# jenkinsm13/julia-spira

Measured on AMD Instinct MI355X. Metric: Msamples/sec at 1920x1080 spp=64 depth=8; fraction of HBM roofline, higher is better.
Workload: dtype f64

## Files before the change

julia-spira_amd/csrc/spira_device.h:

```cpp
#pragma once
#include <hip/hip_runtime.h>
#include <stdint.h>
#include <type_traits>
#include "spira_fastdiv.h"

namespace spira {

__device__ __forceinline__ float sqrt_rn(float x) { return __builtin_sqrtf(x); }
__device__ __forceinline__ double sqrt_rn(double x) { return __builtin_sqrt(x); }

constexpr int kBlock = 256;
#ifndef SPIRA_WAVES_F32
#define SPIRA_WAVES_F32 5
#endif
#ifndef SPIRA_WAVES_F64
#define SPIRA_WAVES_F64 4
#endif
#define SPIRA_WAVES_PER_SIMD(T) (sizeof(T) == 8 ? SPIRA_WAVES_F64 : SPIRA_WAVES_F32)
constexpr uint32_t kMaxTries = 64;

template <class T> struct Vec { T x, y, z; };

template <class T> __device__ __forceinline__ Vec<T> mk(T x, T y, T z) { Vec<T> r; r.x = x; r.y = y; r.z = z; return r; }
template <class T> __device__ __forceinline__ Vec<T> operator+(Vec<T> a, Vec<T> b) { return mk<T>(a.x + b.x, a.y + b.y, a.z + b.z); }
// ... 1117 lines not shown
            if (have) {
                const uint32_t *kw = reinterpret_cast<const uint32_t *>(&s_rnd[e]);
                k.hA = kw[0]; k.hB = kw[1]; k.hBr = (k.hB << 16) | (k.hB >> 16);
            }
            while (__any(have)) {
                bool done = false;
                if (have) {
                    T u0, u1, u2;
                    rng3<T>(k, t, u0, u1, u2, (T)(1.0 / 1048576.0));
                    Vec<T> c = mk<T>(u0, u1, u2) - mk<T>(1, 1, 1);
                    done = dot(c, c) < (T)1.0;
                    if (!done && t == kMaxTries) { c = mk<T>(0, 0, 0); done = true; }
                    if (done) { Pack4<T> w; w.x = c.x; w.y = c.y; w.z = c.z; w.w = 0; s_rnd[e] = w; }
                    ++t;
                }
                const unsigned long long m = __ballot(done);
                if (done) {
                    e = next + __popcll(m & lt_mask); t = 1;
                    have = e < n_list;
                    if (have) {
                        const uint32_t *kw = reinterpret_cast<const uint32_t *>(&s_rnd[e]);
                        k.hA = kw[0]; k.hB = kw[1]; k.hBr = (k.hB << 16) | (k.hB >> 16);
                    }
                }
                next += (uint32_t)__popcll(m);
            }
        }
        wave_lds_sync();
#pragma unroll
        for (int r = 0; r < R; ++r) {
            const bool alive = pend[r].kind != kDead;
            const unsigned long long m = __ballot(alive);
            if (alive) {
                Vec<T> rnd = mk<T>(0, 0, 0);
                if (pend[r].kind != kMirror) { const Pack4<T> w = s_rnd[ent[r]]; rnd = mk<T>(w.x, w.y, w.z); }
                const Vec<T> nd = segment_back<T>(o[r], pend[r], rnd);
                const uint32_t dst = region + fill + __popcll(m & lt_mask);
                Pack4<T> A, B; Pack2<T> C;
                A.x = o[r].x; A.y = o[r].y; A.z = o[r].z; A.w = nd.x;
                B.x = nd.y; B.y = nd.z; B.z = beta[r].x; B.w = beta[r].y;
                C.x = beta[r].z; C.y = Bits<T>::from_u32(q[r]);
                a.qout.A[dst] = A; a.qout.B[dst] = B; a.qout.C[dst] = C;
            }
            fill += (uint32_t)__popcll(m);
        }
        wave_lds_sync();
    }
    for (int sft = 32; sft > 0; sft >>= 1) { n_rmw += __shfl_down(n_rmw, sft); n_seg += __shfl_down(n_seg, sft); n_store += __shfl_down(n_store, sft); }
    if (lane == 0) {
        if (scatter) a.cnt_out[wid] = fill;
        a.blk_stats[4 * wid] = n_seg;
        a.blk_stats[4 * wid + 1] = n_rmw;
        a.blk_stats[4 * wid + 2] = n_store;
        a.blk_stats[4 * wid + 3] = FIRST ? 0u : n_seg;
    }
}

template <class T> struct PathArgs {
    SceneGlobal<T> scene;
    RenderConst<T> rc;
    RayQueue<T> q[2];
    uint32_t *qref[2];
    uint2 *qkey[2];
    uint32_t cam_consts;
    Pack3<T> *L;
    uint32_t *blk_stats;
    uint32_t cap;
    uint32_t pass;
    uint32_t n_first;
    uint32_t dense_pct;
    Pack4<T> *mesh_list;
    uint32_t mesh_min_batch;
    uint32_t refill_free;
    uint32_t mesh_mode;
    uint32_t *mesh_count;
    uint32_t resume_k, resume_nw;
    uint32_t *redo;
    uint32_t redo_only;
    Stats *stats;
    Pack4<T> *accum;
    FastDiv fd_keff;
    uint32_t k_eff;
    uint32_t accum_first;
};

#ifndef SPIRA_RESOLVE_RUN
#define SPIRA_RESOLVE_RUN 4
#endif
__device__ __forceinline__ uint32_t owned_pixel(uint32_t w, uint32_t nw, uint32_t l) {
    constexpr uint32_t kRun = SPIRA_RESOLVE_RUN;
    static_assert(64 % kRun == 0, "a run length divides the wave");
    return ((l / kRun) * nw + w) * kRun + l % kRun;
}

template <class T>
__device__ __forceinline__ void resolve_pixel(Pack4<T> *accum, const Pack3<T> *L, uint32_t tile_pixels, uint32_t k_eff, bool first_pass, uint32_t p) {
    Pack4<T> acc;
    if (first_pass) { acc.x = 0; acc.y = 0; acc.z = 0; acc.w = 0; } else acc = accum[p];
    uint32_t s = 0;
    for (; s + 8 <= k_eff; s += 8) {
        Pack3<T> l[8];
#pragma unroll
        for (int k = 0; k < 8; ++k) l[k] = L[(size_t)(s + k) * tile_pixels + p];
#pragma unroll
        for (int k = 0; k < 8; ++k) { acc.x = acc.x + l[k].x; acc.y = acc.y + l[k].y; acc.z = acc.z + l[k].z; }
    }
    for (; s < k_eff; ++s) {
        const Pack3<T> l = L[(size_t)s * tile_pixels + p];
        acc.x = acc.x + l.x; acc.y = acc.y + l.y; acc.z = acc.z + l.z;
    }
    accum[p] = acc;
}

__device__ __forceinline__ float pack_qref(uint32_t q, uint32_t, float) { return __uint_as_float(q); }
__device__ __forceinline__ double pack_qref(uint32_t q, uint32_t ref, double) { return __longlong_as_double((long long)((unsigned long long)q | ((unsigned long long)ref << 32))); }
__device__ __forceinline__ uint32_t unpack_q(float w) { return __float_as_uint(w); }
__device__ __forceinline__ uint32_t unpack_q(double w) { return (uint32_t)(unsigned long long)__double_as_longlong(w); }
__device__ __forceinline__ uint32_t unpack_ref(double w) { return (uint32_t)((unsigned long long)__double_as_longlong(w) >> 32); }

#ifdef SPIRA_MESH_STATS
__device__ unsigned long long g_mesh_dbg[32];
#define MESH_STAT(...) __VA_ARGS__
#else
#define MESH_STAT(...)
#endif

#ifndef SPIRA_CARRY_KEY
#define SPIRA_CARRY_KEY 1
#endif
#ifndef SPIRA_WAVES_B_F32
#define SPIRA_WAVES_B_F32 4
#endif
#ifndef SPIRA_WAVES_B_F64
#define SPIRA_WAVES_B_F64 SPIRA_WAVES_F64
#endif
#ifndef SPIRA_WAVES_PATH_F32
#define SPIRA_WAVES_PATH_F32 6
#endif
template <class T, int R, bool BVH, bool EXT, bool SPEC, int MODE = 0, bool TRI = true>
__global__ __launch_bounds__(kBlock, MODE == 2 ? (sizeof(T) == 8 ? SPIRA_WAVES_B_F64 : SPIRA_WAVES_B_F32) : (sizeof(T) == 4 ? SPIRA_WAVES_PATH_F32 : SPIRA_WAVES_F64)) void k_path(const PathArgs<T> a) {
    extern __shared__ __attribute__((aligned(32))) unsigned char lds_raw[];
    constexpr uint32_t WPB = kBlock / 64, SUB = 64 * R;
    constexpr bool kRefArray = sizeof(T) == 4;
    constexpr bool kCarry = SPIRA_CARRY_KEY && !BVH && !EXT;
    constexpr uint32_t kStageShift = 25, kRefMask = (1u << kStageShift) - 1u;
    const uint32_t lane = threadIdx.x & 63, wave = threadIdx.x >> 6;
    const uint32_t NW = gridDim.x * WPB, wid = blockIdx.x * WPB + wave;
    const RenderConst<T> &rc = a.rc;
    using Pol = typename std::conditional<SPEC, SpecDiv, ExactDiv>::type;
    Pol pol;
    if (!SPEC && a.redo_only) {
        uint32_t any = 0;
        for (uint32_t w = 0; w < WPB; ++w) any |= a.redo[blockIdx.x * WPB + w];
        if (!any) return;
    }
    T *cam_lds = reinterpret_cast<T *>(lds_raw + scene_lds_bytes<T>(a.scene.n_spheres, a.scene.n_materials, a.scene.n_triangles) + WPB * SUB * sizeof(Pack4<T>));
    if (threadIdx.x < 12) {
        const Vec<T> *cv = threadIdx.x < 3 ? &rc.cam_origin : (threadIdx.x < 6 ? &rc.cam_llc : (threadIdx.x < 9 ? &rc.cam_hor : &rc.cam_ver));
        const uint32_t cc = threadIdx.x % 3;
        cam_lds[threadIdx.x] = cc == 0 ? cv->x : (cc == 1 ? cv->y : cv->z);
    }
    Pack4<T> *cam_sph = reinterpret_cast<Pack4<T> *>(reinterpret_cast<unsigned char *>(cam_lds) + 128);
    constexpr bool kCam = !EXT;
    if (kCam && MODE != 2 && a.cam_consts)
        for (uint32_t i = threadIdx.x; i < a.scene.n_spheres; i += blockDim.x) {
            const T *sp = a.scene.spheres5 + 5 * (size_t)i;
            const Vec<T> oc = rc.cam_origin - mk<T>(sp[0], sp[1], sp[2]);
            Pack4<T> k; k.x = oc.x; k.y = oc.y; k.z = oc.z; k.w = dot(oc, oc) - sp[3] * sp[3];
            cam_sph[i] = k;
        }
    const SceneLds<T> sc = stage_scene<T>(a.scene, lds_raw);
    const PixelDiv<T> pix_div = pixel_divisors<T>(rc);
    if (!SPEC && a.redo_only) {
        if (!a.redo[wid]) return;
        if (lane == 0) atomicAdd(&a.stats->redone_waves, 1ull);
    }
    Pack4<T> *s_rnd = reinterpret_cast<Pack4<T> *>(lds_raw + scene_lds_bytes<T>(a.scene.n_spheres, a.scene.n_materials, a.scene.n_triangles)) + wave * SUB;
    constexpr uint32_t mesh_mode = BVH ? (uint32_t)MODE : 0u;
    const uint32_t kseg = mesh_mode == 2u ? a.resume_k : 1u;
    if (mesh_mode == 2u && wid * kseg >= a.resume_nw) return;
    const uint32_t region = wid * kseg * a.cap;
    const unsigned long long lt_mask = (1ull << lane) - 1ull;
    const uint32_t ref_base = sc.n_spheres + sc.n_triangles;
    const bool mixed = mesh_mode != 0u || rc.max_depth <= 128u;
    const uint32_t dense_pct = mixed ? a.dense_pct : 0u;
    const bool defer = mesh_mode != 0u || (BVH && mixed && a.mesh_list != nullptr);
    Pack4<T> *mlist = a.mesh_list + 3 * (size_t)region;
    uint32_t n_rmw = 0, n_store = 0, n_seg = 0, n_enq = 0, n_park = 0;
    uint32_t n_wtrips = 0, n_ltrips = 0;
    uint32_t n_in = 0;
    const bool own = !BVH && !EXT && !TRI && sizeof(T) == 8 && a.accum != nullptr;
    const uint32_t n_own = own ? 64u * a.k_eff : 0u;
    const uint32_t n_sub_first = own ? (n_own + SUB - 1) / SUB : (a.n_first + SUB - 1) / SUB;

    auto park = [&](uint32_t slot_i, const Vec<T> o_, const Vec<T> d_, const Vec<T> beta_, T closest_, uint32_t q_, int prim_, uint32_t stage_hit) {
        Pack4<T> A, B, C;
        A.x = o_.x; A.y = o_.y; A.z = o_.z; A.w = d_.x;
        B.x = d_.y; B.y = d_.z; B.z = beta_.x; B.w = beta_.y;
        C.x = beta_.z; C.y = closest_; C.z = Bits<T>::from_u32(q_); C.w = Bits<T>::from_u32((uint32_t)(prim_ + 1) | (stage_hit << kStageShift));
        mlist[3 * (size_t)slot_i] = A; mlist[3 * (size_t)slot_i + 1] = B; mlist[3 * (size_t)slot_i + 2] = C;
    };
    uint32_t mfill = 0;
    constexpr int kMaxSeg = 16;
    uint32_t pfx[kMaxSeg + 1];
    bool segmented = false;
    {
        uint32_t cnt = 0;
        if (mesh_mode == 2u && lane < kseg && wid * kseg + lane < a.resume_nw) cnt = a.mesh_count[wid * kseg + lane];
        pfx[0] = 0;
#pragma unroll
        for (int j = 0; j < kMaxSeg; ++j) pfx[j + 1] = pfx[j] + (uint32_t)__builtin_amdgcn_readlane((int)cnt, j);
        if (mesh_mode == 2u) { mfill = pfx[kMaxSeg]; segmented = true; }
    }
    const uint32_t first_sub = own ? 0u : (mesh_mode == 1u ? (wid % a.resume_k) * (NW / a.resume_k) + wid / a.resume_k : wid);
    const uint32_t sub_step = own ? 1u : NW;
    MESH_STAT(unsigned long long dbg_t0 = __builtin_readcyclecounter(); unsigned long long dbg_sess = 0, dbg_walk = 0; uint32_t dbg_ns = 0, dbg_ws = 0, dbg_ls = 0, dbg_rf = 0, dbg_rays = 0, dbg_rounds = 0, dbg_ws1 = 0, dbg_ls1 = 0, dbg_h[4] = {0, 0, 0, 0};)
    for (uint32_t round = 0; ; ++round) {
        MESH_STAT(++dbg_rounds;)
        const bool first = mesh_mode != 2u && round == 0;
        const RayQueue<T> qin = a.q[(round + 1) & 1], qout = a.q[round & 1];
        const uint32_t *rin = a.qref[(round + 1) & 1];
        uint32_t *rout = a.qref[round & 1];
        const uint2 *kin = a.qkey[(round + 1) & 1];
        uint2 *kout = a.qkey[round & 1];
        const uint32_t limit = first ? (own ? n_own : a.n_first) : n_in;
        const uint32_t n_sub = first ? n_sub_first : (n_in + SUB - 1) / SUB;
        uint32_t fill = 0;
        for (uint32_t sub = first ? first_sub : 0u; sub < n_sub; sub += first ? sub_step : 1u) {
            Vec<T> o[R], beta[R];
            Pending<T> pend[R];
            ExtState<T> ex[R];
            uint32_t q[R], ent[R], stg[R], ref[R];
            uint32_t ka[R], kb[R];
            bool valid[R];
#pragma unroll
            for (int r = 0; r < R; ++r) {
                const uint32_t idx = sub * SUB + r * 64 + lane;
                valid[r] = false; stg[r] = round; ref[r] = 0; q[r] = 0; ka[r] = 0; kb[r] = 0;
                pend[r].kind = kDead; pend[r].rough = 0; pend[r].v = mk<T>(0, 0, 0);
                o[r] = mk<T>(0, 0, 0); beta[r] = mk<T>(1, 1, 1);
                bool parked = false; T park_t = 0; int park_prim = -1;
                uint32_t qf = idx;
                bool in = idx < limit;
                if (own && first) {
                    const uint32_t t = idx / SPIRA_RESOLVE_RUN, run = fastdiv(t, a.fd_keff);
                    const uint32_t px = owned_pixel(wid, NW, run * SPIRA_RESOLVE_RUN + idx % SPIRA_RESOLVE_RUN);
                    qf = (t - run * a.k_eff) * rc.tile_pixels + px;
                    in = in && px < rc.tile_pixels;
                }
                if (in) {
                    if (first) {
                        uint32_t pixel, sample, pi, pj;
                        Vec<T> d;
                        q[r] = qf;
                        path_of<T>(rc, qf, a.pass, pi, pj, pixel, sample);
                        if (kCarry) { ka[r] = mix32(rc.sA + pixel) ^ (sample << 8); kb[r] = mix32(rc.sB ^ pixel) + (sample << 8); }
                        camera_ray_lds<T>(rc, cam_lds, pix_div, pi, pj, pixel, sample, o[r], d, pol);
                        if (EXT) { ex[r].flags = rc.flags; if (rc.flags & kExtSpectral) beta[r] = ext_wavelength<T>(sc, rc.sA, rc.sB, pixel, sample, ex[r]); }
                        T t; uint32_t slot = 0;
                        int prim;
                        if (defer) {
                            if (kCam && a.cam_consts) closest_hit_local<T, Pol, TRI, true>(sc, o[r], d, (T)0.001, t, prim, pol, cam_sph);
                            else closest_hit_local<T, Pol, TRI>(sc, o[r], d, (T)0.001, t, prim, pol);
                            parked = mesh_box_hit<T>(sc, o[r], d, t);
                        } else if (kCam && !BVH && a.cam_consts) { closest_hit_local<T, Pol, TRI, true>(sc, o[r], d, (T)0.001, t, prim, pol, cam_sph); }
                        else prim = closest_hit<T, BVH, Pol, TRI>(sc, o[r], d, (T)0.001, t, slot, pol);
                        ++n_seg;
                        if (parked) { park_t = t; park_prim = prim; pend[r].v = d; }
                        else if (prim < 0) {
                            const Vec<T> c = sky_term_x<T, EXT>(d, beta[r], &ex[r]);
                            Pack3<T> l; l.x = c.x; l.y = c.y; l.z = c.z;
                            a.L[qf] = l;
                            ++n_store;
                        } else {
                            valid[r] = true;
                            o[r] = o[r] + d * t;
                            ref[r] = (BVH && prim >= (int)ref_base) ? ref_base + slot : (uint32_t)prim;
                            pend[r].v = d;
                        }
                    } else {
                        const Pack4<T> A = qin.A[region + idx], B = qin.B[region + idx];
                        const Pack2<T> C = qin.C[region + idx];
                        o[r] = mk<T>(A.x, A.y, A.z);
                        pend[r].v = mk<T>(A.w, B.x, B.y);
                        beta[r] = mk<T>(B.z, B.w, C.x);
                        q[r] = unpack_q(C.y);
                        uint32_t w;
                        if constexpr (kRefArray) w = rin[region + idx]; else w = unpack_ref(C.y);
                        if (mixed) { stg[r] = w >> kStageShift; ref[r] = w & kRefMask; } else ref[r] = w;
                        if (kCarry) { const uint2 k = kin[region + idx]; ka[r] = k.x; kb[r] = k.y; }
                        valid[r] = true;
                    }
                }
                if (defer && first) {
                    const unsigned long long mp = __ballot(parked);
                    if (parked) park(mfill + __popcll(mp & lt_mask), o[r], pend[r].v, beta[r], park_t, q[r], park_prim, 0u);
                    mfill += (uint32_t)__popcll(mp); n_park += (uint32_t)__popcll(mp);
                }
            }
            while (true) {
                uint32_t n_list = 0, n_valid = 0;
#pragma unroll
                for (int r = 0; r < R; ++r) {
                    bool want = false;
                    RngKey key;
                    const Vec<T> d = pend[r].v;
                    pend[r].kind = kDead;
                    if (valid[r]) {
                        uint32_t pixel = 0, sample = 0, pi, pj;
                        const bool scatter = stg[r] + 1 < rc.max_depth;
                        int prim = (int)ref[r]; uint32_t slot = 0;
                        if (BVH && ref[r] >= ref_base) { prim = (int)ref_base; slot = ref[r] - ref_base; }
                        const uint32_t qi = q[r] & 0x7FFFFFFFu;
                        const bool has_l = (q[r] >> 31) != 0;
                        if (EXT) {
                            path_of<T>(rc, qi, a.pass, pi, pj, pixel, sample);
                            ex[r].flags = rc.flags;
                            if (rc.flags & kExtSpectral) (void)ext_wavelength<T>(sc, rc.sA, rc.sB, pixel, sample, ex[r]);
                        }
                        Vec<T> contrib;
                        const bool has_contrib = shade_hit<T, BVH, EXT, Pol, TRI>(sc, o[r], d, prim, slot, beta[r], scatter, contrib, pend[r], &ex[r], pol);
                        if (has_contrib) {
                            Pack3<T> l; l.x = contrib.x; l.y = contrib.y; l.z = contrib.z;
                            if (has_l) { const Pack3<T> l0 = a.L[qi]; l.x = l0.x + contrib.x; l.y = l0.y + contrib.y; l.z = l0.z + contrib.z; ++n_rmw; }
                            else ++n_store;
                            a.L[qi] = l;
                            q[r] |= 0x80000000u;
                        } else if (!scatter && !has_l) {
                            Pack3<T> l; l.x = 0; l.y = 0; l.z = 0;
                            a.L[qi] = l;
                            ++n_store;
                        }
                        want = (pend[r].kind == kDiffuse || pend[r].kind == kSpecRough);
                        if (want || (EXT && pend[r].kind == kDielectric)) {
                            if (kCarry && mixed) {
                                key.hA = mix32(ka[r] ^ stg[r]); key.hB = mix32(kb[r] + stg[r]); key.hBr = (key.hB << 16) | (key.hB >> 16);
                            } else {
                                if (!EXT) path_of<T>(rc, qi, a.pass, pi, pj, pixel, sample);
                                key = rng_key(rc.sA, rc.sB, pixel, sample, stg[r]);
                            }
                            if (EXT && pend[r].kind == kDielectric) dielectric_resolve<T>(pend[r], d, key);
                        }
                    }
                    const unsigned long long mv = __ballot(pend[r].kind != kDead);
                    n_valid += (uint32_t)__popcll(mv);
                    const unsigned long long m = __ballot(want);
                    if (want) {
                        ent[r] = n_list + __popcll(m & lt_mask);
                        uint32_t *kw = reinterpret_cast<uint32_t *>(&s_rnd[ent[r]]);
                        kw[0] = key.hA; kw[1] = key.hB;
                    }
                    n_list += (uint32_t)__popcll(m);
                }
                if (n_valid == 0) break;
                wave_lds_sync();
// ... 237 lines not shown
                    if (prim < 0) {
                        const uint32_t qi = q_ & 0x7FFFFFFFu;
                        ExtState<T> ex1; ex1.flags = rc.flags; ex1.bR = 0; ex1.bG = 0; ex1.bB = 0;
                        if (EXT && (rc.flags & kExtSpectral)) {
                            uint32_t pi, pj, pixel, sample;
                            path_of<T>(rc, qi, a.pass, pi, pj, pixel, sample);
                            (void)ext_wavelength<T>(sc, rc.sA, rc.sB, pixel, sample, ex1);
                        }
                        const Vec<T> c = sky_term_x<T, EXT>(d_, beta_, &ex1);
                        Pack3<T> l; l.x = c.x; l.y = c.y; l.z = c.z;
                        if (q_ >> 31) { const Pack3<T> l0 = a.L[qi]; l.x = l0.x + c.x; l.y = l0.y + c.y; l.z = l0.z + c.z; ++n_rmw; }
                        else ++n_store;
                        a.L[qi] = l;
                    } else {
                        const Vec<T> hp = o_ + d_ * closest;
                        const uint32_t w_ = ((prim >= (int)ref_base) ? ref_base + slot : (uint32_t)prim) | (stage_hit << kStageShift);
                        const uint32_t dst = region + fill + __popcll(mh & lt_mask);
                        Pack4<T> A, B; Pack2<T> C;
                        A.x = hp.x; A.y = hp.y; A.z = hp.z; A.w = d_.x;
                        B.x = d_.y; B.y = d_.z; B.z = beta_.x; B.w = beta_.y;
                        C.x = beta_.z; C.y = pack_qref(q_, w_, (T)0);
                        qout.A[dst] = A; qout.B[dst] = B; qout.C[dst] = C;
                        if constexpr (kRefArray) rout[dst] = w_;
                    }
                }
                fill += (uint32_t)__popcll(mh);
                finished = false;
                const unsigned long long mf = __ballot(!walking);
                const uint32_t take = min((uint32_t)__popcll(mf), mfill - next);
                if (!walking && (uint32_t)__popcll(mf & lt_mask) < take) {
                    const uint32_t e = next + (uint32_t)__popcll(mf & lt_mask);
                    const Pack4<T> *ent = mlist + 3 * (size_t)e;
                    if (segmented) {
                        uint32_t seg = 0, off = e;
#pragma unroll
                        for (int j = 1; j < kMaxSeg; ++j) if (e >= pfx[j]) { seg = (uint32_t)j; off = e - pfx[j]; }
                        ent = a.mesh_list + 3 * ((size_t)(wid * kseg + seg) * a.cap + off);
                    }
                    const Pack4<T> A = ent[0], B = ent[1], C = ent[2];
                    o_ = mk<T>(A.x, A.y, A.z); d_ = mk<T>(A.w, B.x, B.y); beta_ = mk<T>(B.z, B.w, C.x);
                    closest = C.y;
                    q_ = Bits<T>::to_u32(C.z);
                    const uint32_t pw = Bits<T>::to_u32(C.w);
                    prim = (int)(pw & kRefMask) - 1;
                    stage_hit = pw >> kStageShift;
                    slot = 0;
                    T t0;
                    if (bvh8_enter<T>(sc, o_, d_, closest, ry, t0)) { bvh8_begin<T>(wk, ry, t0, (T)0.001, sc.bvh_root[2].w); walking = true; }
                    else finished = true;
                }
                next += take;
                if (!__any(walking)) { if (__any(finished)) continue; break; }
                const bool more = next < mfill;
                MESH_STAT(++dbg_rf; const unsigned long long dbg_w0 = __builtin_readcyclecounter();)
                uint32_t n_now = (uint32_t)__popcll(__ballot(walking));
                while (true) {
                    ++n_wtrips; n_ltrips += n_now;
                    MESH_STAT(++dbg_ws; { const uint32_t nl = (uint32_t)__popcll(__ballot(walking)); dbg_ls += nl; if (segmented) { ++dbg_ws1; dbg_ls1 += nl; } ++dbg_h[nl <= 8 ? 0 : (nl <= 24 ? 1 : (nl <= 48 ? 2 : 3))]; })
                    if (walking && !bvh8_step<T, kLdsStack>(sc, wk, ry, o_, d_, (T)0.001, (int)ref_base, closest, prim, slot, lstack, stack, lane)) { walking = false; finished = true; }
                    const uint32_t n_walk = (uint32_t)__popcll(__ballot(walking));
                    n_now = n_walk;
                    if (n_walk == 0 || (more && 64u - n_walk >= a.refill_free)) break;
                }

                MESH_STAT(dbg_walk += __builtin_readcyclecounter() - dbg_w0;)
            }
            }
            mfill = 0;
            segmented = false;
            MESH_STAT(dbg_sess += __builtin_readcyclecounter() - dbg_s0;)
        }
        n_in = fill;
        n_enq += fill;
        if (n_in == 0 && (mfill == 0 || mesh_mode == 1u)) break;
        __builtin_amdgcn_fence(__ATOMIC_RELEASE, "workgroup");
        __builtin_amdgcn_fence(__ATOMIC_ACQUIRE, "workgroup");
    }
    for (int sft = 32; sft > 0; sft >>= 1) { n_rmw += __shfl_down(n_rmw, sft); n_seg += __shfl_down(n_seg, sft); n_store += __shfl_down(n_store, sft); }
    const bool again = SPEC && __any(outside_window<T>(pol));
    if (own && !again && !(SPEC && a.redo_only == 2u)) {
        __builtin_amdgcn_fence(__ATOMIC_RELEASE, "workgroup");
        __builtin_amdgcn_fence(__ATOMIC_ACQUIRE, "workgroup");
        const uint32_t px = owned_pixel(wid, NW, lane);
        if (px < rc.tile_pixels) resolve_pixel<T>(a.accum, a.L, rc.tile_pixels, a.k_eff, a.accum_first != 0, px);
        const uint32_t seg = __shfl(n_seg, 0), rmw = __shfl(n_rmw, 0), sto = __shfl(n_store, 0);
        if (lane < 4) {
            unsigned long long *f = lane == 0 ? &a.stats->segments : (lane == 1 ? &a.stats->rays_enqueued : (lane == 2 ? &a.stats->radiance_rmw : &a.stats->radiance_store));
            atomicAdd(f, (unsigned long long)(lane == 0 ? seg : (lane == 1 ? n_enq : (lane == 2 ? rmw : sto))));
        }
    }
    MESH_STAT(if (lane == 0) { unsigned long long *g = g_mesh_dbg + (mesh_mode == 2u ? 16 : 0);
                               atomicAdd(&g[0], __builtin_readcyclecounter() - dbg_t0); atomicAdd(&g[1], dbg_sess); atomicAdd(&g[2], (unsigned long long)dbg_ns);
                               atomicAdd(&g[3], (unsigned long long)dbg_ws); atomicAdd(&g[4], (unsigned long long)dbg_ls); atomicAdd(&g[5], (unsigned long long)dbg_rf);
                               atomicAdd(&g[6], (unsigned long long)dbg_rays); atomicAdd(&g[7], (unsigned long long)dbg_rounds); atomicAdd(&g[9], dbg_walk); atomicAdd(&g[10], 1ull); atomicAdd(&g[11], (unsigned long long)dbg_ws1); atomicAdd(&g[12], (unsigned long long)dbg_ls1);
                               atomicAdd(&g[8], (unsigned long long)dbg_h[0]); atomicAdd(&g[13], (unsigned long long)dbg_h[1]); atomicAdd(&g[14], (unsigned long long)dbg_h[2]); atomicAdd(&g[15], (unsigned long long)dbg_h[3]); })
    if (lane == 0) {
        if (mesh_mode == 2u) {
            const uint32_t row = 4 * wid * kseg;
            a.blk_stats[row] += n_seg; a.blk_stats[row + 1] += n_rmw; a.blk_stats[row + 2] += n_store; a.blk_stats[row + 3] += n_enq;
        } else {
            a.blk_stats[4 * wid] = n_seg;
            a.blk_stats[4 * wid + 1] = n_rmw;
            a.blk_stats[4 * wid + 2] = n_store;
            a.blk_stats[4 * wid + 3] = n_enq;
            if (mesh_mode == 1u) a.mesh_count[wid] = mfill;
        }
        if (SPEC) a.redo[wid] = again ? 1u : 0u;
        if (BVH && n_park && !again && !(SPEC && a.redo_only == 2u)) atomicAdd(&a.stats->rays_parked, (unsigned long long)n_park);
        if (BVH && mesh_mode != 1u && n_wtrips && !again && !(SPEC && a.redo_only == 2u)) { atomicAdd(&a.stats->mesh_wave_trips, (unsigned long long)n_wtrips); atomicAdd(&a.stats->mesh_lane_trips, (unsigned long long)n_ltrips); }
    }
}

template <class T, bool BVH, bool EXT>
__global__ __launch_bounds__(kBlock) void k_mega(const BounceArgs<T> a) {
    extern __shared__ __attribute__((aligned(32))) unsigned char lds_raw[];
    const SceneLds<T> sc = stage_scene<T>(a.scene, lds_raw);
    const RenderConst<T> &rc = a.rc;
    unsigned long long nseg = 0;
    const uint32_t stride = gridDim.x * kBlock;
    uint32_t idx = blockIdx.x * kBlock + threadIdx.x;
    bool fresh = true;
    uint32_t pixel = 0, sample = 0, b = 0;
    Vec<T> o = mk<T>(0, 0, 0), d = mk<T>(0, 0, 1), beta = mk<T>(1, 1, 1), Lacc = mk<T>(0, 0, 0);
    ExtState<T> ex; ex.flags = rc.flags; ex.bR = 0; ex.bG = 0; ex.bB = 0;
    while (idx < a.n_first) {
        if (fresh) {
            uint32_t pi, pj;
            path_of<T>(rc, idx, a.pass, pi, pj, pixel, sample);
            camera_ray<T>(rc, pi, pj, pixel, sample, o, d);
            beta = mk<T>(1, 1, 1); Lacc = mk<T>(0, 0, 0); b = 0;
            if (EXT && (rc.flags & kExtSpectral)) beta = ext_wavelength<T>(sc, rc.sA, rc.sB, pixel, sample, ex);
            fresh = false;
        }
        Vec<T> contrib; T t_hit;
        SegInfo si = trace_segment<T, BVH, EXT>(sc, rc, o, d, beta, pixel, sample, b, b + 1 < rc.max_depth, contrib, t_hit, &ex);
        ++nseg;
        if (b == 0) { if (si.has_contrib) Lacc = contrib; }
        else if (si.has_contrib) Lacc = Lacc + contrib;
        ++b;
        if (!si.alive || b == rc.max_depth) {
            Pack3<T> l; l.x = Lacc.x; l.y = Lacc.y; l.z = Lacc.z;
            a.L[idx] = l;
            idx += stride;
            fresh = true;
        }
    }
    for (int sft = 32; sft > 0; sft >>= 1) nseg += __shfl_down(nseg, sft);
    if ((threadIdx.x & 63) == 0 && nseg) atomicAdd(&a.stats->segments, nseg);
}

template <class T, bool BVH, bool EXT>
__global__ __launch_bounds__(64) void k_trace(const BounceArgs<T> a, const uint32_t *ijs, uint32_t n_paths, int *prims, T *ts,
                                              T *dirs, T *radiance) {
    extern __shared__ __attribute__((aligned(32))) unsigned char lds_raw[];
    const SceneLds<T> sc = stage_scene<T>(a.scene, lds_raw);
    const RenderConst<T> &rc = a.rc;
    uint32_t p = blockIdx.x * blockDim.x + threadIdx.x;
    if (p >= n_paths) return;
    uint32_t i = ijs[3 * p], j = ijs[3 * p + 1], sample = ijs[3 * p + 2];
    uint32_t pixel = (j - 1) * rc.width + (i - 1);
    Vec<T> o, d, beta = mk<T>(1, 1, 1), Lacc = mk<T>(0, 0, 0);
    camera_ray<T>(rc, i, j, pixel, sample, o, d);
    ExtState<T> ex; ex.flags = rc.flags; ex.bR = 0; ex.bG = 0; ex.bB = 0;
    if (EXT && (rc.flags & kExtSpectral)) beta = ext_wavelength<T>(sc, rc.sA, rc.sB, pixel, sample, ex);
    for (uint32_t b = 0; b < rc.max_depth; ++b) {
        Vec<T> contrib; T t_hit;
        Vec<T> dir_in = d;
// ... 761 lines not shown
```

julia-spira_amd/csrc/spira_hip.hip:

```cpp
#include <hip/hip_runtime.h>
#include <sys/mman.h>
#include <rccl/rccl.h>
#include <dlfcn.h>

#include <algorithm>
#include <atomic>
#include <chrono>
#include <cmath>
#include <cstdio>
#include <cstdlib>
#include <cstring>
#include <condition_variable>
#include <mutex>
#include <new>
#include <string>
#include <thread>
#include <vector>

#include "../../include/spira_hip.h"
#include "../../include/spira_spd.h"
#include "spira_device.h"
#include "spira_bvh.h"
#include "spira_validate.h"

// ... 493 lines not shown
                  const spira_params *p, spira::SceneGlobal<T> &g, bool reuse = false) {
    if (h) { scene_pointers<T>(h->store, g); return 0; }
    if (reuse) { scene_pointers<T>(c.scene, g); return 0; }
    const uint32_t nt = triangles10 ? p->n_triangles : 0;
    if (int rc = scene_upload<T>(c.scene, st, c.have_done ? c.ev_done : nullptr, spheres5, materials8, triangles10, p->n_spheres, p->n_materials, nt)) return rc;
    scene_pointers<T>(c.scene, g);
    return 0;
}

template <class T>
int attach_spd(Ctx &c, hipStream_t st, const spira_params *p, spira::SceneGlobal<T> &g) {
    g.spd = nullptr;
    if (!(p->flags & SPIRA_EXT_SPECTRAL)) return 0;
    DevBuf &b = sizeof(T) == 4 ? c.spd32 : c.spd64;
    if (!b.p) {
        static_assert(SPIRA_SPD_N == spira::kSpdN && SPIRA_SPD_ROWS == spira::kSpdRows, "SPD table shape");
        T host[SPIRA_SPD_ROWS * SPIRA_SPD_N];
        for (int r = 0; r < SPIRA_SPD_ROWS; ++r)
            for (int i = 0; i < SPIRA_SPD_N; ++i) host[r * SPIRA_SPD_N + i] = (T)spira_spd_table[r][i];
        if (int rc = b.ensure(sizeof host)) return rc;
        HIP_TRY(hipMemcpy(b.p, host, sizeof host, hipMemcpyHostToDevice));
    }
    (void)st;
    g.spd = (const T *)b.p;
    return 0;
}

template <class T>
int check_handle(const spira_scene *h) {
    if (!h || h->magic != kSceneMagic) return fail(SPIRA_E_INVALID, "scene handle is NULL or was destroyed");
    if (h->prec != (int)sizeof(T)) return fail(SPIRA_E_INVALID, "scene handle was created in the other precision");
    if (h->device != tl_device) return fail(SPIRA_E_INVALID, "scene handle belongs to another device (spira_set_device)");
    return 0;
}

struct PathPlan {
    uint64_t waves = 0;
    uint64_t packets = 0;
    uint64_t batch = 0;
    bool queues = false;
    bool mesh = false;
    bool two_pass = false;
    bool spec = false;
};
template <class T>
int ensure_path_plan(Ctx &c, const PathPlan &pl) {
    using P4 = spira::Pack4<T>;
    using P2 = spira::Pack2<T>;
    if (pl.queues)
        for (int i = 0; i < 2; ++i) {
            if (int rc = c.qA[i].ensure(pl.packets * sizeof(P4))) return rc;
            if (int rc = c.qB[i].ensure(pl.packets * sizeof(P4))) return rc;
            if (int rc = c.qC[i].ensure(pl.packets * sizeof(P2))) return rc;
            if (sizeof(T) == 4) { if (int rc = c.qR[i].ensure(pl.packets * sizeof(uint32_t))) return rc; }
            if (!pl.mesh) { if (int rc = c.qK[i].ensure(pl.packets * sizeof(uint2))) return rc; }
        }
    if (pl.mesh) { if (int rc = c.mesh_list.ensure(3 * pl.packets * sizeof(P4))) return rc; }
    if (pl.two_pass) { if (int rc = c.mesh_count.ensure(pl.waves * sizeof(uint32_t))) return rc; }
    if (pl.spec) { if (int rc = c.redo.ensure(pl.waves * sizeof(uint32_t))) return rc; }
    if (int rc = c.blkstats.ensure(pl.waves * 4 * sizeof(uint32_t))) return rc;
    if (int rc = c.L.ensure(pl.batch * sizeof(spira::Pack3<T>))) return rc;
    return c.stats.ensure(sizeof(spira::Stats));
}
template <class T>
int verify_path_args(const Ctx &c, const spira::PathArgs<T> &a, uint32_t first_launch_blocks) {
    using P4 = spira::Pack4<T>;
    using P2 = spira::Pack2<T>;
    const uint64_t nw = (uint64_t)first_launch_blocks * (spira::kBlock / 64), n = nw * a.cap;
    auto covers = [](const DevBuf &b, const void *ptr, uint64_t bytes) { return ptr == b.p && b.p != nullptr && b.cap >= bytes; };
    const char *bad = nullptr;
    const bool mesh = a.scene.n_bvh_tris != 0;
    if ((uint64_t)a.n_first > n) bad = "the pass does not fit its queue regions";
    if (a.rc.max_depth > 1 || mesh)
        for (int i = 0; i < 2 && !bad; ++i) {
            if (!covers(c.qA[i], a.q[i].A, n * sizeof(P4)) || !covers(c.qB[i], a.q[i].B, n * sizeof(P4)) || !covers(c.qC[i], a.q[i].C, n * sizeof(P2))) bad = "hit queues";
            else if (sizeof(T) == 4 && !covers(c.qR[i], a.qref[i], n * sizeof(uint32_t))) bad = "hit reference arrays";
            else if (!mesh && !covers(c.qK[i], a.qkey[i], n * sizeof(uint2))) bad = "carried RNG keys";
        }
    if (!bad && a.mesh_list && !covers(c.mesh_list, a.mesh_list, 3 * n * sizeof(P4))) bad = "mesh lists";
    if (!bad && a.mesh_mode != 0 && (!a.mesh_list || !covers(c.mesh_count, a.mesh_count, nw * sizeof(uint32_t)) || a.resume_k == 0 || a.resume_k > 16 || nw % a.resume_k != 0 || a.resume_nw != nw))
        bad = "parked-ray counts of a two-launch mesh pass";
    if (!bad && a.redo && !covers(c.redo, a.redo, nw * sizeof(uint32_t))) bad = "redo flags";
    if (!bad && !covers(c.blkstats, a.blk_stats, nw * 4 * sizeof(uint32_t))) bad = "per-wave statistics";
    if (!bad && !covers(c.L, a.L, (uint64_t)a.n_first * sizeof(spira::Pack3<T>))) bad = "per-path radiance";
    if (!bad && !covers(c.stats, a.stats, sizeof(spira::Stats))) bad = "counters";
    if (!bad && a.accum) {
        const uint64_t tp = a.rc.tile_pixels;
        if (!covers(c.accum, a.accum, tp * sizeof(spira::Pack4<T>)) || sizeof(T) != 8 || a.scene.n_triangles || mesh || (a.rc.flags & (SPIRA_EXT_DIELECTRIC | SPIRA_EXT_SPECTRAL)) ||
            a.k_eff == 0 || a.k_eff > 64 || (uint64_t)a.k_eff * tp != a.n_first || 64 * nw < tp || a.cap < 64ull * a.k_eff)
            bad = "pixel-owning pass";
    }
    if (bad) return fail(SPIRA_E_LIMIT, std::string("internal: a workspace is smaller than the launch needs (") + bad + ")");
    return 0;
}

template <class T>
int render_impl(const spira_scene *h, const T *spheres5, const T *materials8, const T *triangles10, const T *camera12, const spira_params *p,
                T *out_hdr, T *out_img, bool out_on_device, void *user_stream,
                bool progressive = false, uint32_t sample0 = 0, uint32_t *rng_states = nullptr, const SlabCtl *slab = nullptr) {
    uint32_t rows = 0;
    const bool cont = slab && slab->index > 0;
    if (!p) return fail(SPIRA_E_INVALID, "params is NULL");
    tl_lds_optin = hipSuccess;
    Lap lap("render");
    if (h) { if (int rc = check_handle<T>(h)) return rc; }
    else if (!cont) { if (int rc = validate_scene<T>(spheres5, materials8, triangles10, p->n_spheres, p->n_materials, triangles10 ? p->n_triangles : 0)) return rc; }
    if (int rc = validate_params(camera12, p, h ? h->store.nt : (triangles10 ? p->n_triangles : 0), &rows)) return rc;
    lap("validate");
    if (!out_hdr && !out_img) return fail(SPIRA_E_INVALID, "both outputs are NULL");
    if (progressive && (uint64_t)sample0 + p->spp > SPIRA_MAX_SPP) return fail(SPIRA_E_LIMIT, "sample0 + spp exceeds 2^24");
    if (progressive && (p->flags & SPIRA_SEM_MASK) == SPIRA_SEM_HYBRID) return fail(SPIRA_E_UNSUPPORTED, "SPIRA_SEM_HYBRID has no accumulate entry (its image is a mean of tone-mapped samples)");
    if (progressive && (p->flags & SPIRA_SEM_MASK) == SPIRA_SEM_METAL && sample0 > 0 && !rng_states)
        return fail(SPIRA_E_INVALID, "SPIRA_SEM_METAL with sample0 > 0 needs rng_states (the LCG states the previous call left); "
                                     "without them every call would replay the samples of the first");
    Ctx *cp = nullptr;
    if (int rc = get_ctx(&cp)) return rc;
    Ctx &c = *cp;
    std::lock_guard<std::recursive_mutex> lock(c.mu);
    hipStream_t st = out_on_device ? (hipStream_t)user_stream : c.stream;
    if (int rc = order_after_previous(c, st)) return rc;
    lap("context");

    const uint32_t W = p->width;
    const uint64_t tile_pixels = (uint64_t)rows * W;
    uint32_t target = p->batch_rays ? p->batch_rays : env_u32("SPIRA_BATCH_RAYS", 160u << 20);
    uint64_t slots64 = std::max<uint64_t>(1, target / tile_pixels);
    slots64 = std::min<uint64_t>(slots64, p->spp);
    slots64 = (p->spp + (p->spp + slots64 - 1) / slots64 - 1) / ((p->spp + slots64 - 1) / slots64);
    if (slots64 * tile_pixels > 0x7FFFFFFFull) return fail(SPIRA_E_LIMIT, "tile too large: rows*width must be < 2^31");
    const uint32_t slots = (uint32_t)slots64;
    const uint64_t batch = slots64 * tile_pixels;
    const uint32_t sem = p->flags & SPIRA_SEM_MASK;
    const bool mega = (p->flags & SPIRA_KERNEL_MASK) == SPIRA_KERNEL_MEGA || sem != SPIRA_SEM_A;
    const bool metal_wavefront = sem == SPIRA_SEM_METAL && (p->flags & SPIRA_KERNEL_MASK) == SPIRA_KERNEL_WAVEFRONT;
    uint64_t metal_launches = 0;
    const bool per_bounce = !mega && (p->flags & SPIRA_KERNEL_MASK) == SPIRA_KERNEL_BOUNCE;
    const bool persistent = !mega && !per_bounce;
    const bool profile = ((p->flags & SPIRA_FLAG_PROFILE) != 0 && per_bounce) || persistent;
    int R = (int)env_u32("SPIRA_R", 2);
    if (R != 1 && R != 2) R = 2;
    if (p->flags & (SPIRA_EXT_DIELECTRIC | SPIRA_EXT_SPECTRAL)) R = 2;

    const uint32_t nt_scene = h ? h->store.nt : (triangles10 ? p->n_triangles : 0);
    const bool mesh_two_pass = persistent && nt_scene > SPIRA_LDS_TRIANGLES && p->max_depth <= 128 && env_u32("SPIRA_DEFER_MESH", 1) && env_u32("SPIRA_MESH_TWO_PASS", 1);
    const uint32_t blocks_per_cu = !persistent ? 16 : ((nt_scene > SPIRA_LDS_TRIANGLES && !mesh_two_pass) ? 4 : 32);
    const uint32_t max_blocks = (uint32_t)c.num_cus * env_u32("SPIRA_BLOCKS_PER_CU", blocks_per_cu);
    const uint32_t wpb = spira::kBlock / 64;
    const uint32_t sub = 64 * R;
    const bool fused = persistent && sizeof(T) == 8 && R == 2 && nt_scene == 0 && (p->flags & (SPIRA_EXT_DIELECTRIC | SPIRA_EXT_SPECTRAL)) == 0 &&
                       slots <= 64 && env_u32("SPIRA_FUSED_RESOLVE", 1) != 0;
    auto geometry = [&](uint64_t n_first, uint32_t &G, uint32_t &cap) {
        if (fused) {
            const uint64_t k = n_first / tile_pixels;
            G = (uint32_t)((tile_pixels + 64 * wpb - 1) / (64 * wpb));
            cap = (uint32_t)((64 * k + sub - 1) / sub * sub);
            return;
        }
        const uint64_t n_sub = (n_first + sub - 1) / sub;
        G = (uint32_t)std::min<uint64_t>((n_sub + wpb - 1) / wpb, max_blocks);
        const uint64_t nw = (uint64_t)G * wpb;
        cap = (uint32_t)(((n_sub + nw - 1) / nw) * sub);
    };
    uint32_t G_max = 0, cap_max = 0;
    geometry(batch, G_max, cap_max);
    const uint64_t q_rays = (uint64_t)cap_max * G_max * wpb;
    if (q_rays > 0xFFFFFFFFull) return fail(SPIRA_E_LIMIT, "pass too large");

    using P4 = spira::Pack4<T>;
    using P2 = spira::Pack2<T>;
    const bool mesh_scene = nt_scene > SPIRA_LDS_TRIANGLES;
    const bool defer_mesh = persistent && mesh_scene && p->max_depth <= 128 && env_u32("SPIRA_DEFER_MESH", 1) != 0;
    PathPlan plan;
    plan.waves = (uint64_t)G_max * wpb; plan.packets = q_rays; plan.batch = batch;
    plan.queues = !mega && (p->max_depth > 1 || (persistent && mesh_scene));
    plan.mesh = defer_mesh; plan.two_pass = defer_mesh && mesh_two_pass; plan.spec = persistent && env_u32("SPIRA_SPEC_DIV", 1) != 0;
    if (persistent) { if (int rc = ensure_path_plan<T>(c, plan)) return rc; }
    else {
        if (plan.queues)
            for (int i = 0; i < 2; ++i) {
                if (int rc = c.qA[i].ensure(q_rays * sizeof(P4))) return rc;
                if (int rc = c.qB[i].ensure(q_rays * sizeof(P4))) return rc;
                if (int rc = c.qC[i].ensure(q_rays * sizeof(P2))) return rc;
            }
        if (sem != SPIRA_SEM_HYBRID) { if (int rc = c.L.ensure(batch * sizeof(spira::Pack3<T>))) return rc; }
        if (per_bounce) { if (int rc = c.counts.ensure((size_t)(p->max_depth + 2) * G_max * wpb * sizeof(uint32_t))) return rc; }
        if (int rc = c.blkstats.ensure((size_t)(per_bounce ? p->max_depth + 1 : 1) * G_max * wpb * 4 * sizeof(uint32_t))) return rc;
        if (int rc = c.stats.ensure(sizeof(spira::Stats))) return rc;
    }
    if (int rc = c.accum.ensure(tile_pixels * sizeof(P4))) return rc;

    lap("workspaces");
    spira::BounceArgs<T> a{};
    if (int rc = acquire_scene<T>(c, st, h, spheres5, materials8, triangles10, p, a.scene, cont)) return rc;
    if (int rc = attach_spd<T>(c, st, p, a.scene)) return rc;
    lap("scene");
    const bool scene_moderate = h ? h->store.moderate : c.scene.moderate;
    fill_const<T>(a.rc, camera12, p, rows, slots);
    if (!fastdiv_selfcheck(a.rc.tile_pixels, (uint32_t)batch) || !fastdiv_selfcheck(a.rc.width, a.rc.tile_pixels) ||
        !fastdiv_selfcheck(a.rc.stripe_h ? a.rc.stripe_h : 1, rows))
        return fail(SPIRA_E_LIMIT, "internal: fast division self-check failed");
    a.L = (spira::Pack3<T> *)c.L.p;
    a.stats = (spira::Stats *)c.stats.p;

    const size_t lds = spira::scene_lds_bytes<T>(a.scene.n_spheres, a.scene.n_materials, a.scene.n_triangles);
    const uint32_t n_pass = (p->spp + slots - 1) / slots;

    T *d_hdr = out_hdr, *d_img = out_img;
    if (!out_on_device) {
        size_t plane3 = 3 * tile_pixels * sizeof(T);
        if (int rc = c.out_tmp.ensure(2 * plane3)) return rc;
        d_hdr = out_hdr ? (T *)c.out_tmp.p : nullptr;
        d_img = out_img ? (T *)((char *)c.out_tmp.p + plane3) : nullptr;
    }

    size_t n_prof = 0;
    if (profile) {
        n_prof = (size_t)n_pass * (persistent ? 1 : std::max<uint32_t>(p->max_depth, 1)) * 2;
        if (int rc = profile_events(c, (cont ? c.ev_used : 0) + n_prof)) return rc;
    }
    if (!cont) {
        c.ev_used = 0;
        c.ev_mid_used = 0;
        HIP_TRY(hipMemsetAsync(c.stats.p, 0, sizeof(spira::Stats), st));
        HIP_TRY(hipEventRecord(c.ev_start, st));
    }
    uint64_t launches = 0;

    a.rc.sample0 = progressive ? sample0 : 0;
    uint32_t *d_rng = nullptr;
    if (progressive) {
        const uint32_t lblocks = std::min<uint32_t>((uint32_t)((tile_pixels + spira::kBlock - 1) / spira::kBlock), max_blocks);
        if (!out_on_device) HIP_TRY(hipMemcpyAsync(d_hdr, out_hdr, 3 * tile_pixels * sizeof(T), hipMemcpyHostToDevice, st));
        hipLaunchKernelGGL((spira::k_load_accum<T>), dim3(lblocks), dim3(spira::kBlock), 0, st, (P4 *)c.accum.p, (const T *)d_hdr, (uint32_t)tile_pixels);
        ++launches;
        if (rng_states) {
            d_rng = rng_states;
            if (!out_on_device) {
                if (int rc = c.rng.ensure(tile_pixels * sizeof(uint32_t))) return rc;
                d_rng = (uint32_t *)c.rng.p;
                if (sample0 > 0) HIP_TRY(hipMemcpyAsync(d_rng, rng_states, tile_pixels * sizeof(uint32_t), hipMemcpyHostToDevice, st));
            }
        }
    }

    if (p->max_depth == 0) {
        if (!progressive) HIP_TRY(hipMemsetAsync(c.accum.p, 0, tile_pixels * sizeof(P4), st));
    } else if (sem == SPIRA_SEM_HYBRID) {
        const uint64_t P = tile_pixels;
        if (P > 0xFFFFFFFFull / 2) return fail(SPIRA_E_LIMIT, "image too large for SPIRA_SEM_HYBRID");
        if (int rc = c.hyb_state.ensure(12 * P * sizeof(T))) return rc;
        if (int rc = c.hyb_mat.ensure(P * sizeof(uint32_t))) return rc;
        if (int rc = c.rng.ensure(P * sizeof(uint32_t))) return rc;
        const size_t n_flags = (size_t)p->spp * (p->max_depth + 1);
        if (int rc = c.hyb_flags.ensure(n_flags * sizeof(uint32_t))) return rc;
        HIP_TRY(hipMemsetAsync(c.hyb_flags.p, 0, n_flags * sizeof(uint32_t), st));
        HIP_TRY(hipMemsetAsync(c.accum.p, 0, P * sizeof(P4), st));
// ... 56 lines not shown
        hipLaunchKernelGGL(spira::k_fold_stats, dim3(1), dim3(64), 0, st, (const uint32_t *)c.blkstats.p, Gm * wpb, (spira::Stats *)c.stats.p);
        launches += 2;
        metal_launches = 1;
    } else if (sem == SPIRA_SEM_METAL) {
        uint32_t blocks = std::min<uint32_t>((uint32_t)((tile_pixels + spira::kBlock - 1) / spira::kBlock), max_blocks);
        a.pass = 0; a.n_first = (uint32_t)tile_pixels;
        const int resume = progressive ? (sample0 > 0 ? 3 : 1) : 0;
        int spec = (int)env_u32("SPIRA_SPEC_DIV", 1);
        if (spec == 1 && !(scene_moderate && spira::camera_scale_moderate<T>(camera12))) spec = 0;
        if (spec == 3) spec = 1;
        if (resume) spec = 0;
        if (spec) {
            if (int rc = c.redo.ensure((size_t)blocks * wpb * sizeof(uint32_t))) return rc;
            uint32_t *redo = (uint32_t *)c.redo.p;
            launch_lds(spira::k_variant_metal<T, true>, dim3(blocks), dim3(spira::kBlock), lds, st, a, (P4 *)c.accum.p, d_rng, resume, redo, spec == 2 ? 2 : 0);
            launch_lds(spira::k_variant_metal<T, false>, dim3(blocks), dim3(spira::kBlock), lds, st, a, (P4 *)c.accum.p, d_rng, resume, redo, 1);
            launches += 2;
        } else {
            launch_lds(spira::k_variant_metal<T, false>, dim3(blocks), dim3(spira::kBlock), lds, st, a, (P4 *)c.accum.p, d_rng, resume, (uint32_t *)nullptr, 0);
            ++launches;
        }
    } else {
        for (uint32_t pass = 0; pass < n_pass; ++pass) {
            const uint32_t k_eff = std::min(slots, p->spp - pass * slots);
            const uint32_t n_first = (uint32_t)((uint64_t)k_eff * tile_pixels);
            a.pass = pass;
            a.n_first = n_first;
            uint32_t G = 0, stat_rows = 0;
            if (sem == SPIRA_SEM_CPU) {
                uint32_t blocks = std::min<uint32_t>((n_first + spira::kBlock - 1) / spira::kBlock, max_blocks);
                int spec = (int)env_u32("SPIRA_SPEC_DIV", 1);
                if (spec == 1 && !(scene_moderate && spira::camera_scale_moderate<T>(camera12))) spec = 0;
                if (spec == 3) spec = 1;
                if (spec) {
                    if (int rc = c.redo.ensure((size_t)max_blocks * wpb * sizeof(uint32_t))) return rc;
                    uint32_t *redo = (uint32_t *)c.redo.p;
                    launch_lds(spira::k_variant_cpu<T, true>, dim3(blocks), dim3(spira::kBlock), lds, st, a, redo, spec == 2 ? 2 : 0);
                    launch_lds(spira::k_variant_cpu<T, false>, dim3(blocks), dim3(spira::kBlock), lds, st, a, redo, 1);
                    launches += 2;
                } else {
                    launch_lds(spira::k_variant_cpu<T, false>, dim3(blocks), dim3(spira::kBlock), lds, st, a, (uint32_t *)nullptr, 0);
                    ++launches;
                }
            } else if (mega) {
                uint32_t blocks = std::min<uint32_t>((n_first + spira::kBlock - 1) / spira::kBlock, max_blocks);
                const bool ext = (p->flags & (SPIRA_EXT_DIELECTRIC | SPIRA_EXT_SPECTRAL)) != 0;
                if (a.scene.n_bvh_tris) { if (ext) launch_lds(spira::k_mega<T, true, true>, dim3(blocks), dim3(spira::kBlock), lds, st, a); else launch_lds(spira::k_mega<T, true, false>, dim3(blocks), dim3(spira::kBlock), lds, st, a); }
                else { if (ext) launch_lds(spira::k_mega<T, false, true>, dim3(blocks), dim3(spira::kBlock), lds, st, a); else launch_lds(spira::k_mega<T, false, false>, dim3(blocks), dim3(spira::kBlock), lds, st, a); }
                ++launches;
            } else if (persistent) {
                spira::PathArgs<T> pa{};
                pa.scene = a.scene; pa.rc = a.rc; pa.L = a.L; pa.pass = pass; pa.n_first = n_first;
                pa.dense_pct = std::min<uint32_t>(env_u32("SPIRA_DENSE_PCT", 70), 100);
                pa.mesh_list = plan.mesh ? (P4 *)c.mesh_list.p : nullptr;
                geometry(n_first, G, pa.cap);
                stat_rows = G * wpb;
                for (int i = 0; i < 2; ++i) {
                    pa.q[i] = {(P4 *)c.qA[i].p, (P4 *)c.qB[i].p, (P2 *)c.qC[i].p};
                    pa.qref[i] = (uint32_t *)c.qR[i].p;
                    pa.qkey[i] = (uint2 *)c.qK[i].p;
                }
                pa.blk_stats = (uint32_t *)c.blkstats.p;
                pa.stats = (spira::Stats *)c.stats.p;
                int spec = (int)env_u32("SPIRA_SPEC_DIV", 1);
                if (spec == 1 && !(scene_moderate && spira::camera_scale_moderate<T>(camera12))) spec = 0;
                if (spec == 3) spec = 1;
                if (spec) pa.redo = (uint32_t *)c.redo.p;
                pa.mesh_mode = 0; pa.mesh_count = nullptr; pa.resume_k = 1; pa.resume_nw = 0;
                pa.mesh_min_batch = std::max<uint32_t>(1, env_u32("SPIRA_MESH_MIN_BATCH", 128));
                pa.refill_free = std::min<uint32_t>(64, std::max<uint32_t>(1, env_u32("SPIRA_MESH_REFILL", 16)));
                size_t lds_a = lds + (size_t)wpb * sub * sizeof(P4) + 128;
                pa.cam_consts = (env_u32("SPIRA_CAM_CONSTS", 1) && a.scene.n_spheres && lds_a + (size_t)a.scene.n_spheres * sizeof(P4) <= (size_t)160 * 1024) ? 1u : 0u;
                if (pa.cam_consts) lds_a += (size_t)a.scene.n_spheres * sizeof(P4);
                if (plan.two_pass) {
                    pa.mesh_mode = 1; pa.mesh_count = (uint32_t *)c.mesh_count.p;
                    const uint32_t nw = G * wpb, fat = std::max<uint32_t>(1, (uint32_t)c.num_cus * env_u32("SPIRA_MESH_FAT_WAVES_PER_CU", 16));
                    uint32_t k = 16;
                    while (k > 1 && (nw % k != 0 || nw / k < fat)) k >>= 1;
                    pa.resume_k = k; pa.resume_nw = nw;
                }
                if (fused) {
                    pa.accum = (P4 *)c.accum.p; pa.k_eff = k_eff; pa.fd_keff = spira::fastdiv_make(k_eff);
                    pa.accum_first = (pass == 0 && !progressive) ? 1u : 0u;
                }
                if (int rc = verify_path_args<T>(c, pa, G)) return rc;
                HIP_TRY(hipEventRecord(c.ev_pool[c.ev_used++], st));
                if (int rc = launch_path<T>(R, dim3(G), lds_a, st, pa, spec)) return rc;
                if (int rc = lds_optin_failed()) return rc;
                launches += (spec && R == 2) ? 2 : 1;
                if (pa.mesh_mode == 1) {
                    if (c.ev_mid.size() <= c.ev_mid_used) {
                        hipEvent_t e;
                        HIP_TRY(hipEventCreate(&e));
                        c.ev_mid.push_back(e); c.ev_mid_end.push_back(0);
                    }
                    HIP_TRY(hipEventRecord(c.ev_mid[c.ev_mid_used], st));
                    c.ev_mid_end[c.ev_mid_used++] = c.ev_used;
                    spira::PathArgs<T> pb = pa;
                    pb.mesh_mode = 2; pb.n_first = 0;
                    const uint32_t nwb = pa.resume_nw / pa.resume_k;
                    launch_path_resume_entry<T>(R, dim3((nwb + wpb - 1) / wpb), lds_a, st, pb);
                    if (int rc = lds_optin_failed()) return rc;
                    ++launches;
                }
                HIP_TRY(hipEventRecord(c.ev_pool[c.ev_used++], st));
            } else {
                geometry(n_first, G, a.cap);
                stat_rows = p->max_depth * G * wpb;
                const size_t nw = (size_t)G * wpb;
                for (uint32_t b = 0; b < p->max_depth; ++b) {
                    a.bounce = b;
                    int qi = b & 1;
                    a.qout = {(P4 *)c.qA[qi].p, (P4 *)c.qB[qi].p, (P2 *)c.qC[qi].p};
                    a.qin = {(P4 *)c.qA[qi ^ 1].p, (P4 *)c.qB[qi ^ 1].p, (P2 *)c.qC[qi ^ 1].p};
                    a.cnt_in = (const uint32_t *)c.counts.p + (size_t)b * nw;
                    a.cnt_out = (uint32_t *)c.counts.p + (size_t)(b + 1) * nw;
                    a.blk_stats = (uint32_t *)c.blkstats.p + (size_t)b * nw * 4;
                    if (profile) HIP_TRY(hipEventRecord(c.ev_pool[c.ev_used++], st));
                    const size_t lds_b = lds + (size_t)wpb * sub * sizeof(P4);
                    if (b == 0) launch_bounce<T, true>(R, dim3(G), lds_b, st, a);
                    else launch_bounce<T, false>(R, dim3(G), lds_b, st, a);
                    if (int rc = lds_optin_failed()) return rc;
                    if (profile) HIP_TRY(hipEventRecord(c.ev_pool[c.ev_used++], st));
                    ++launches;
                }
            }
            if (fused) continue;
            uint32_t rblocks = std::min<uint32_t>((uint32_t)((tile_pixels + spira::kBlock - 1) / spira::kBlock), max_blocks);
            hipLaunchKernelGGL((spira::k_resolve<T>), dim3(rblocks), dim3(spira::kBlock), 0, st, (P4 *)c.accum.p, (const spira::Pack3<T> *)c.L.p,
                               (uint32_t)tile_pixels, k_eff, (pass == 0 && !progressive) ? 1 : 0, mega ? (const uint32_t *)nullptr : (const uint32_t *)c.blkstats.p,
                               stat_rows, (spira::Stats *)c.stats.p);
            ++launches;
        }
    }
    {
        uint32_t fblocks = std::min<uint32_t>((uint32_t)((tile_pixels + spira::kBlock - 1) / spira::kBlock), max_blocks);
        if (progressive)
            hipLaunchKernelGGL((spira::k_finalize<T>), dim3(fblocks), dim3(spira::kBlock), 0, st, (const P4 *)c.accum.p, (uint32_t)tile_pixels,
                               1u, (uint32_t)SPIRA_POST_NONE, d_hdr, (T *)nullptr);
        else
            hipLaunchKernelGGL((spira::k_finalize<T>), dim3(fblocks), dim3(spira::kBlock), 0, st, (const P4 *)c.accum.p, (uint32_t)tile_pixels,
                               p->spp, sem == SPIRA_SEM_HYBRID ? (uint32_t)SPIRA_POST_NONE : (p->flags & SPIRA_POST_MASK), d_hdr, d_img);
        ++launches;
    }
    if (progressive && rng_states && !out_on_device)
        HIP_TRY(hipMemcpyAsync(rng_states, d_rng, tile_pixels * sizeof(uint32_t), hipMemcpyDeviceToHost, st));
    if (int rc = lds_optin_failed()) return rc;
    HIP_TRY(hipGetLastError());
    HIP_TRY(hipEventRecord(c.ev_stop, st));
    HIP_TRY(hipMemcpyAsync(c.h_stats, c.stats.p, sizeof(spira::Stats), hipMemcpyDeviceToHost, st));
    lap("enqueue");

    if (!cont) c.last = spira_counters{};
    c.last.samples += (uint64_t)p->spp * tile_pixels;
    c.last.passes += p->max_depth ? n_pass : 0;
    c.last.launches += launches;
    c.last.bounce_launches += metal_launches ? metal_launches : ((mega || !p->max_depth) ? 0 : (uint64_t)n_pass * (persistent ? 1 : p->max_depth));
    c.last_valid = true;
    c.last_pending = true;
    c.last_stream = st;

    if (!out_on_device) {
        void *const dst[2] = {out_hdr, out_img};
        const void *const src[2] = {d_hdr, d_img};
        if (int rc = copy_out(c, st, dst, src, 3 * tile_pixels * sizeof(T))) return rc;
    }
// ... 740 lines not shown
```

Measured before the change: 26070.

## Store per-path radiance in wave-private contiguous blocks for pixel-owning resolve

```diff
diff --git a/julia-spira_amd/csrc/spira_device.h b/julia-spira_amd/csrc/spira_device.h
--- a/julia-spira_amd/csrc/spira_device.h
+++ b/julia-spira_amd/csrc/spira_device.h
@@ -1223,6 +1223,7 @@
     FastDiv fd_keff;
     uint32_t k_eff;
     uint32_t accum_first;
+    uint32_t l_private;
 };
 
 #ifndef SPIRA_RESOLVE_RUN
@@ -1248,6 +1249,25 @@
     }
     for (; s < k_eff; ++s) {
         const Pack3<T> l = L[(size_t)s * tile_pixels + p];
+        acc.x = acc.x + l.x; acc.y = acc.y + l.y; acc.z = acc.z + l.z;
+    }
+    accum[p] = acc;
+}
+template <class T>
+__device__ __forceinline__ void resolve_pixel_run(Pack4<T> *accum, const Pack3<T> *Lp, uint32_t k_eff, bool first_pass, uint32_t p) {
+    constexpr uint32_t kRun = SPIRA_RESOLVE_RUN;
+    Pack4<T> acc;
+    if (first_pass) { acc.x = 0; acc.y = 0; acc.z = 0; acc.w = 0; } else acc = accum[p];
+    uint32_t s = 0;
+    for (; s + 8 <= k_eff; s += 8) {
+        Pack3<T> l[8];
+#pragma unroll
+        for (int k = 0; k < 8; ++k) l[k] = Lp[(s + k) * kRun];
+#pragma unroll
+        for (int k = 0; k < 8; ++k) { acc.x = acc.x + l[k].x; acc.y = acc.y + l[k].y; acc.z = acc.z + l[k].z; }
+    }
+    for (; s < k_eff; ++s) {
+        const Pack3<T> l = Lp[s * kRun];
         acc.x = acc.x + l.x; acc.y = acc.y + l.y; acc.z = acc.z + l.z;
     }
     accum[p] = acc;
@@ -1333,6 +1353,8 @@
     const bool own = !BVH && !EXT && !TRI && sizeof(T) == 8 && a.accum != nullptr;
     const uint32_t n_own = own ? 64u * a.k_eff : 0u;
     const uint32_t n_sub_first = own ? (n_own + SUB - 1) / SUB : (a.n_first + SUB - 1) / SUB;
+    const bool priv = kCarry && own && a.l_private != 0;
+    const uint32_t l_base = priv ? wid * n_own : 0u;
 
     auto park = [&](uint32_t slot_i, const Vec<T> o_, const Vec<T> d_, const Vec<T> beta_, T closest_, uint32_t q_, int prim_, uint32_t stage_hit) {
         Pack4<T> A, B, C;
@@ -1389,11 +1411,12 @@
                     qf = (t - run * a.k_eff) * rc.tile_pixels + px;
                     in = in && px < rc.tile_pixels;
                 }
+                const uint32_t ql = priv ? l_base + idx : qf;
                 if (in) {
                     if (first) {
                         uint32_t pixel, sample, pi, pj;
                         Vec<T> d;
-                        q[r] = qf;
+                        q[r] = ql;
                         path_of<T>(rc, qf, a.pass, pi, pj, pixel, sample);
                         if (kCarry) { ka[r] = mix32(rc.sA + pixel) ^ (sample << 8); kb[r] = mix32(rc.sB ^ pixel) + (sample << 8); }
                         camera_ray_lds<T>(rc, cam_lds, pix_div, pi, pj, pixel, sample, o[r], d, pol);
@@ -1411,7 +1434,7 @@
                         else if (prim < 0) {
                             const Vec<T> c = sky_term_x<T, EXT>(d, beta[r], &ex[r]);
                             Pack3<T> l; l.x = c.x; l.y = c.y; l.z = c.z;
-                            a.L[qf] = l;
+                            a.L[ql] = l;
                             ++n_store;
                         } else {
                             valid[r] = true;
@@ -1815,7 +1838,10 @@
         __builtin_amdgcn_fence(__ATOMIC_RELEASE, "workgroup");
         __builtin_amdgcn_fence(__ATOMIC_ACQUIRE, "workgroup");
         const uint32_t px = owned_pixel(wid, NW, lane);
-        if (px < rc.tile_pixels) resolve_pixel<T>(a.accum, a.L, rc.tile_pixels, a.k_eff, a.accum_first != 0, px);
+        if (px < rc.tile_pixels) {
+            if (priv) resolve_pixel_run<T>(a.accum, a.L + l_base + (lane / SPIRA_RESOLVE_RUN) * a.k_eff * SPIRA_RESOLVE_RUN + lane % SPIRA_RESOLVE_RUN, a.k_eff, a.accum_first != 0, px);
+            else resolve_pixel<T>(a.accum, a.L, rc.tile_pixels, a.k_eff, a.accum_first != 0, px);
+        }
         const uint32_t seg = __shfl(n_seg, 0), rmw = __shfl(n_rmw, 0), sto = __shfl(n_store, 0);
         if (lane < 4) {
             unsigned long long *f = lane == 0 ? &a.stats->segments : (lane == 1 ? &a.stats->rays_enqueued : (lane == 2 ? &a.stats->radiance_rmw : &a.stats->radiance_store));
diff --git a/julia-spira_amd/csrc/spira_hip.hip b/julia-spira_amd/csrc/spira_hip.hip
--- a/julia-spira_amd/csrc/spira_hip.hip
+++ b/julia-spira_amd/csrc/spira_hip.hip
@@ -599,7 +599,8 @@
         bad = "parked-ray counts of a two-launch mesh pass";
     if (!bad && a.redo && !covers(c.redo, a.redo, nw * sizeof(uint32_t))) bad = "redo flags";
     if (!bad && !covers(c.blkstats, a.blk_stats, nw * 4 * sizeof(uint32_t))) bad = "per-wave statistics";
-    if (!bad && !covers(c.L, a.L, (uint64_t)a.n_first * sizeof(spira::Pack3<T>))) bad = "per-path radiance";
+    const uint64_t l_entries = a.l_private ? std::max<uint64_t>(a.n_first, 64ull * nw * a.k_eff) : a.n_first;
+    if (!bad && !covers(c.L, a.L, l_entries * sizeof(spira::Pack3<T>))) bad = "per-path radiance";
     if (!bad && !covers(c.stats, a.stats, sizeof(spira::Stats))) bad = "counters";
     if (!bad && a.accum) {
         const uint64_t tp = a.rc.tile_pixels;
@@ -607,6 +608,7 @@
             a.k_eff == 0 || a.k_eff > 64 || (uint64_t)a.k_eff * tp != a.n_first || 64 * nw < tp || a.cap < 64ull * a.k_eff)
             bad = "pixel-owning pass";
     }
+    if (!bad && a.l_private && (!a.accum || !SPIRA_CARRY_KEY || a.rc.max_depth > 128 || l_entries > 0x80000000ull)) bad = "wave-private radiance blocks";
     if (bad) return fail(SPIRA_E_LIMIT, std::string("internal: a workspace is smaller than the launch needs (") + bad + ")");
     return 0;
 }
@@ -678,8 +680,10 @@
         const uint64_t nw = (uint64_t)G * wpb;
         cap = (uint32_t)(((n_sub + nw - 1) / nw) * sub);
     };
+    const bool l_private_wanted = fused && SPIRA_CARRY_KEY && p->max_depth <= 128 && env_u32("SPIRA_PRIVATE_L", 1) != 0;
     uint32_t G_max = 0, cap_max = 0;
     geometry(batch, G_max, cap_max);
+    const bool l_private = l_private_wanted && 64ull * G_max * (spira::kBlock / 64) * slots <= 0x7FFFFFFFull;
     const uint64_t q_rays = (uint64_t)cap_max * G_max * wpb;
     if (q_rays > 0xFFFFFFFFull) return fail(SPIRA_E_LIMIT, "pass too large");
 
@@ -688,7 +692,8 @@
     const bool mesh_scene = nt_scene > SPIRA_LDS_TRIANGLES;
     const bool defer_mesh = persistent && mesh_scene && p->max_depth <= 128 && env_u32("SPIRA_DEFER_MESH", 1) != 0;
     PathPlan plan;
-    plan.waves = (uint64_t)G_max * wpb; plan.packets = q_rays; plan.batch = batch;
+    plan.waves = (uint64_t)G_max * wpb; plan.packets = q_rays;
+    plan.batch = l_private ? std::max<uint64_t>(batch, 64ull * G_max * wpb * slots) : batch;
     plan.queues = !mega && (p->max_depth > 1 || (persistent && mesh_scene));
     plan.mesh = defer_mesh; plan.two_pass = defer_mesh && mesh_two_pass; plan.spec = persistent && env_u32("SPIRA_SPEC_DIV", 1) != 0;
     if (persistent) { if (int rc = ensure_path_plan<T>(c, plan)) return rc; }
@@ -911,6 +916,7 @@
                 if (fused) {
                     pa.accum = (P4 *)c.accum.p; pa.k_eff = k_eff; pa.fd_keff = spira::fastdiv_make(k_eff);
                     pa.accum_first = (pass == 0 && !progressive) ? 1u : 0u;
+                    pa.l_private = l_private ? 1u : 0u;
                 }
                 if (int rc = verify_path_args<T>(c, pa, G)) return rc;
                 HIP_TRY(hipEventRecord(c.ev_pool[c.ev_used++], st));
```

Measured after the change: 27450 (median of 6 runs). +5.3%, better.
